# Tariq-Abuhashim/semantic-slam

Hardware: AMD Instinct MI355X
Metric: Mvoxels/sec integrated, 512³ grid @ 640×480 depth; achieved HBM GB/s %peak (higher is better)
Workload: dtype f32

## Files before the change

### include/tsdf_hip_diag.h

```cpp
#ifndef TSDF_HIP_DIAG_H
#define TSDF_HIP_DIAG_H

#include "tsdf_hip.h"

#ifdef __cplusplus
extern "C" {
#endif


int tsdf_integrate_sequence_timed(tsdf_volume *vol, const float *depth_dev, const float *cam2world,
                                  int32_t n_frames, float *elapsed_ms);

int tsdf_integrate_frames_timed(tsdf_volume *vol, const float *const *depth_dev, const uint8_t *const *masks_dev,
                                const float *cam2world, int32_t n_frames, float *elapsed_ms);


int tsdf_probe_graph_replay(tsdf_volume *vol, const float *depth_dev, const float *cam2world, int32_t n_frames,
                            int32_t iters, float *ms_launches, float *ms_graph);

int tsdf_probe_stream(tsdf_volume *vol, int32_t non_temporal, int32_t n_iters, float *elapsed_ms);


int tsdf_selftest_fastdiv(int32_t device, uint64_t seed, uint64_t n_samples, float fx, float cx,
                          uint64_t *mismatches, float first_bad[4]);

int tsdf_selftest_fastdiv_band(int32_t device, uint64_t seed, uint64_t n_samples, uint64_t *mismatches,
                               float first_bad[4]);

int tsdf_selftest_round(int32_t device, uint64_t *mismatches, float first_bad[4]);

int tsdf_selftest_tile_tables(int32_t device, const float *depth_dev, const uint8_t *mask_dev, int32_t im_height,
                              int32_t im_width, float max_depth, uint64_t *mismatches);


int32_t tsdf_frames_per_launch(const tsdf_volume *vol);
int tsdf_shortcut_stats(tsdf_volume *vol, int32_t enable, uint64_t counts_out[3]);
int tsdf_brick_list_stats(tsdf_volume *vol, uint64_t counts_out[4]);
int tsdf_classification_info(tsdf_volume *vol, double info_out[2]);

int tsdf_last_cam2base(const tsdf_volume *vol, float out[16]);


int tsdf_set_kernel_variant(tsdf_volume *vol, int32_t variant);

int tsdf_set_brick_shape(tsdf_volume *vol, int32_t quads, int32_t rows, int32_t slices);
int tsdf_brick_shape(const tsdf_volume *vol, int32_t shape_out[3]);
int tsdf_default_brick_shape(const tsdf_config *cfg, int32_t shape_out[3]);

#ifdef __cplusplus
}
#endif
#endif
```

### semantic_slam_amd/capi.py

```python
import ctypes as C
import os

import numpy as np

_PKG = os.path.dirname(os.path.abspath(__file__))
LIB_PATH = os.environ.get("TSDF_HIP_LIB") or os.path.join(_PKG, "libtsdf_hip.so")

ABI_SYMBOLS = [
    "tsdf_config_default", "tsdf_create", "tsdf_destroy", "tsdf_reset", "tsdf_integrate",
    "tsdf_integrate_u16", "tsdf_convert_depth_u16", "tsdf_set_deferral",
    "tsdf_integrate_device", "tsdf_integrate_cam2base", "tsdf_integrate_masked_device",
    "tsdf_integrate_frames_device",
    "tsdf_sync", "tsdf_download", "tsdf_copy_slices", "tsdf_upload", "tsdf_refresh_summary", "tsdf_device_ptrs", "tsdf_slab_voxels", "tsdf_frames_per_launch", "tsdf_shortcut_stats", "tsdf_brick_list_stats", "tsdf_classification_info",
    "tsdf_get_config", "tsdf_last_cam2base", "tsdf_set_stream", "tsdf_get_stream",
    "tsdf_count_surface", "tsdf_extract_surface", "tsdf_extract_crossings", "tsdf_extract_mesh", "tsdf_save_mesh_ply", "tsdf_save_mesh_welded_ply", "tsdf_save_ply", "tsdf_save_bin", "tsdf_load_bin", "tsdf_save_state", "tsdf_load_state",
    "tsdf_integrate_sequence_timed", "tsdf_integrate_frames_timed", "tsdf_probe_graph_replay", "tsdf_probe_stream", "tsdf_selftest_fastdiv", "tsdf_selftest_fastdiv_band", "tsdf_selftest_round", "tsdf_selftest_tile_tables", "tsdf_set_kernel_variant", "tsdf_set_brick_shape", "tsdf_brick_shape", "tsdf_default_brick_shape", "tsdf_last_error",
    "tsdf_version", "tsdf_multiply_matrix", "tsdf_invert_matrix",
    "tsdf_labels_enable", "tsdf_compose_labels", "tsdf_integrate_labels_device", "tsdf_integrate_frames_labels_device",
    "tsdf_download_labels",
    "tsdf_colour_enable", "tsdf_integrate_colour_device", "tsdf_integrate_rgbd", "tsdf_download_colour",
    "tsdf_raycast_params_default", "tsdf_raycast_device", "tsdf_raycast", "tsdf_batch_raycast_device",
    "tsdf_track_params_default", "tsdf_track", "tsdf_track_system",
    "tsdf_fuse_params_default", "tsdf_fuse_volume",
    "tsdf_associate_params_default", "tsdf_associate_count", "tsdf_associate_assign", "tsdf_batch_associate",
    "tsdf_segment_params_default", "tsdf_segmenter_create", "tsdf_segmenter_destroy", "tsdf_segmenter_set_stream",
    "tsdf_segment_depth_device", "tsdf_segment_refine_masks_device", "tsdf_segment_frame",
    "tsdf_object_origin", "tsdf_batch_create", "tsdf_batch_destroy", "tsdf_batch_size", "tsdf_batch_volume",
    "tsdf_batch_integrate_device", "tsdf_batch_sync",
    "tsdf_group_create", "tsdf_group_destroy", "tsdf_group_size", "tsdf_group_voxels", "tsdf_group_volume",
    "tsdf_group_integrate", "tsdf_group_integrate_frames", "tsdf_group_set_deferral", "tsdf_group_sync", "tsdf_group_reset", "tsdf_group_download",
    "tsdf_group_extract_surface", "tsdf_group_extract_crossings", "tsdf_group_extract_mesh",
    "tsdf_group_save_ply", "tsdf_group_save_mesh_ply", "tsdf_group_save_bin",
]
DIAG_SYMBOLS = [
    "tsdf_integrate_sequence_timed", "tsdf_integrate_frames_timed",
    "tsdf_probe_graph_replay", "tsdf_probe_stream",
    "tsdf_selftest_fastdiv", "tsdf_selftest_fastdiv_band", "tsdf_selftest_round", "tsdf_selftest_tile_tables",
    "tsdf_shortcut_stats", "tsdf_brick_list_stats", "tsdf_classification_info", "tsdf_frames_per_launch", "tsdf_last_cam2base",
    "tsdf_set_kernel_variant", "tsdf_set_brick_shape", "tsdf_brick_shape", "tsdf_default_brick_shape",
]


class TsdfError(RuntimeError):
    pass


SHIPPED_VARIANTS = (0, 1, 3, 7, 8)


def experiments_build():
    return b"+experiments" in load().tsdf_version()


def variants(*wanted):
    exp = experiments_build()
    return [v for v in wanted if v in SHIPPED_VARIANTS or exp]


class TsdfConfig(C.Structure):
    _fields_ = [
        ("im_height", C.c_int32), ("im_width", C.c_int32),
        ("dim_x", C.c_int32), ("dim_y", C.c_int32), ("dim_z", C.c_int32),
        ("z_begin", C.c_int32), ("z_end", C.c_int32),
        ("voxel_size", C.c_float), ("trunc_margin", C.c_float), ("max_depth", C.c_float),
        ("origin", C.c_float * 3), ("cam_K", C.c_float * 9), ("base2world", C.c_float * 16),
        ("device", C.c_int32), ("id", C.c_int32),
    ]


class RaycastParams(C.Structure):
    _fields_ = [
# ... 57 lines not shown
        raise TsdfError(f"{LIB_PATH} not built: run `python -c 'import __graft_entry__ as g; g.build()'` "
                        "(there is no CPU fallback)")
    try:
        import torch
    except ImportError:
        pass
    L = C.CDLL(LIB_PATH)
    vp, f32p, i64p = C.c_void_p, C.POINTER(C.c_float), C.POINTER(C.c_int64)
    L.tsdf_config_default.argtypes = [C.POINTER(TsdfConfig), C.c_int32, C.c_int32]
    L.tsdf_create.argtypes = [C.POINTER(TsdfConfig), C.POINTER(vp)]
    L.tsdf_destroy.argtypes = [vp]
    L.tsdf_reset.argtypes = [vp]
    L.tsdf_integrate.argtypes = [vp, vp, vp]
    L.tsdf_set_deferral.argtypes = [vp, C.c_int32]
    L.tsdf_integrate_u16.argtypes = [vp, vp, C.c_float, C.c_int32, C.c_int32, vp]
    L.tsdf_convert_depth_u16.argtypes = [vp, vp, vp, C.c_float, C.c_int32, C.c_int32]
    L.tsdf_integrate_device.argtypes = [vp, vp, vp]
    L.tsdf_integrate_cam2base.argtypes = [vp, vp, vp]
    L.tsdf_integrate_masked_device.argtypes = [vp, vp, vp, vp]
    L.tsdf_integrate_frames_device.argtypes = [vp, vp, vp, vp, C.c_int32]
    L.tsdf_sync.argtypes = [vp]
    L.tsdf_download.argtypes = [vp, vp, vp]
    L.tsdf_upload.argtypes = [vp, vp, vp]
    L.tsdf_copy_slices.argtypes = [vp, C.c_int32, C.c_int32, vp, vp]
    L.tsdf_refresh_summary.argtypes = [vp]
    L.tsdf_device_ptrs.argtypes = [vp, C.POINTER(vp), C.POINTER(vp)]
    L.tsdf_slab_voxels.argtypes = [vp]
    L.tsdf_slab_voxels.restype = C.c_int64
    L.tsdf_frames_per_launch.argtypes = [vp]
    L.tsdf_frames_per_launch.restype = C.c_int32
    L.tsdf_shortcut_stats.argtypes = [vp, C.c_int32, vp]
    L.tsdf_classification_info.argtypes = [vp, vp]
    L.tsdf_brick_list_stats.argtypes = [vp, vp]
    L.tsdf_get_config.argtypes = [vp, C.POINTER(TsdfConfig)]
    L.tsdf_last_cam2base.argtypes = [vp, vp]
    L.tsdf_set_stream.argtypes = [vp, vp]
    L.tsdf_get_stream.argtypes = [vp, C.POINTER(vp)]
    L.tsdf_count_surface.argtypes = [vp, C.c_float, i64p]
    L.tsdf_extract_surface.argtypes = [vp, C.c_float, vp, C.c_int64, i64p]
    L.tsdf_extract_crossings.argtypes = [vp, vp, vp, C.c_float, vp, C.c_int64, i64p]
    L.tsdf_extract_mesh.argtypes = [vp, vp, vp, C.c_float, vp, C.c_int64, i64p]
    L.tsdf_save_mesh_ply.argtypes = [vp, C.c_char_p, C.c_float]
    L.tsdf_save_mesh_welded_ply.argtypes = [vp, C.c_char_p, C.c_float]
    L.tsdf_save_ply.argtypes = [vp, C.c_char_p, C.c_float]
    L.tsdf_save_bin.argtypes = [vp, C.c_char_p]
    L.tsdf_load_bin.argtypes = [vp, C.c_char_p]
    L.tsdf_save_state.argtypes = [vp, C.c_char_p]
    L.tsdf_load_state.argtypes = [vp, C.c_char_p]
    L.tsdf_integrate_sequence_timed.argtypes = [vp, vp, vp, C.c_int32, f32p]
    L.tsdf_integrate_frames_timed.argtypes = [vp, vp, vp, vp, C.c_int32, f32p]
    L.tsdf_probe_graph_replay.argtypes = [vp, vp, vp, C.c_int32, C.c_int32, f32p, f32p]
    L.tsdf_probe_stream.argtypes = [vp, C.c_int32, C.c_int32, f32p]
    L.tsdf_selftest_fastdiv.argtypes = [C.c_int32, C.c_uint64, C.c_uint64, C.c_float, C.c_float, C.POINTER(C.c_uint64), f32p]
    L.tsdf_selftest_fastdiv_band.argtypes = [C.c_int32, C.c_uint64, C.c_uint64, C.POINTER(C.c_uint64), f32p]
    L.tsdf_selftest_round.argtypes = [C.c_int32, C.POINTER(C.c_uint64), f32p]
    L.tsdf_selftest_tile_tables.argtypes = [C.c_int32, vp, vp, C.c_int32, C.c_int32, C.c_float, C.POINTER(C.c_uint64)]
    L.tsdf_set_kernel_variant.argtypes = [vp, C.c_int32]
    L.tsdf_set_brick_shape.argtypes = [vp, C.c_int32, C.c_int32, C.c_int32]
    L.tsdf_brick_shape.argtypes = [vp, C.POINTER(C.c_int32)]
    L.tsdf_default_brick_shape.argtypes = [C.POINTER(TsdfConfig), C.POINTER(C.c_int32)]
    L.tsdf_last_error.restype = C.c_char_p
    L.tsdf_version.restype = C.c_char_p
    L.tsdf_multiply_matrix.argtypes = [vp, vp, vp]
    L.tsdf_multiply_matrix.restype = None
    L.tsdf_invert_matrix.argtypes = [vp, vp]
    L.tsdf_labels_enable.argtypes = [vp, C.c_float]
# ... 277 lines not shown

    def close(self):
        if self._h:
            if self._owned:
                self.lib.tsdf_destroy(self._h)
            self._h = C.c_void_p()

    def __enter__(self):
        return self

    def __exit__(self, *exc):
        self.close()

    def __del__(self):
        try:
            self.close()
        except Exception:
            pass

    @property
    def n_voxels(self):
        return int(self.lib.tsdf_slab_voxels(self._h))

    def shortcut_stats(self, enable=True):
        out = (C.c_uint64 * 3)()
        check(self.lib.tsdf_shortcut_stats(self._h, 1 if enable else 0, out), "tsdf_shortcut_stats")
        return tuple(int(x) for x in out)

    def brick_list_stats(self):
        out = (C.c_uint64 * 4)()
        check(self.lib.tsdf_brick_list_stats(self._h, out), "tsdf_brick_list_stats")
        return tuple(int(x) for x in out)

    def classification_info(self):
        out = (C.c_double * 2)()
        check(self.lib.tsdf_classification_info(self._h, out), "tsdf_classification_info")
        return float(out[0]), int(out[1])

    @property
    def frames_per_launch(self):
        return int(self.lib.tsdf_frames_per_launch(self._h))

    @property
    def slab_shape(self):
        c = self.cfg
        return (c.z_end - c.z_begin, c.dim_y, c.dim_x)

    def device_ptrs(self):
        t, w = C.c_void_p(), C.c_void_p()
        check(self.lib.tsdf_device_ptrs(self._h, C.byref(t), C.byref(w)), "tsdf_device_ptrs")
        return t.value, w.value

    def integrate(self, depth_host, cam2world):
        d = _f32(depth_host, self.cfg.im_height * self.cfg.im_width)
        p = _f32(cam2world, 16)
        check(self.lib.tsdf_integrate(self._h, d.ctypes.data, p.ctypes.data), "tsdf_integrate")

    def set_deferral(self, n_frames):
        check(self.lib.tsdf_set_deferral(self._h, n_frames), "tsdf_set_deferral")

    def integrate_u16(self, raw_u16, cam2world, depth_factor=5000.0, row_step=1, col_step=1):
        r = np.ascontiguousarray(raw_u16, dtype=np.uint16).ravel()
        if r.size != self.cfg.im_height * self.cfg.im_width:
            raise ValueError("raw frame size does not match the configured image")
        p = _f32(cam2world, 16)
        check(self.lib.tsdf_integrate_u16(self._h, r.ctypes.data, depth_factor, row_step, col_step, p.ctypes.data),
# ... 440 lines not shown
```

### semantic_slam_amd/csrc/tsdf_capi.hip

```cpp
#include "../../include/tsdf_hip.h"
#include "../../include/tsdf_hip_diag.h"

#include <hip/hip_runtime.h>

#include <algorithm>
#include <cmath>
#include <cstdarg>
#include <cstdio>
#include <cstdlib>
#include <cstring>
#include <new>
#include <string>
#include <unordered_map>
#include <vector>

#include "pose_math.h"
#include "host_derive.h"
#include "host_copy.h"
#include "hip_owned.h"
#include "frame_store.h"
#include "tsdf_kernels.hip.h"
#include "tsdf_multiframe.hip.h"
#include "tsdf_labels.hip.h"
#include "tsdf_colour.hip.h"
// ... 83 lines not shown
    HostPtr<tsdfk::FramePose> h_frames[kStageSlots];
    DevPtr<tsdfk::FramePose> d_frames[kStageSlots];
    Event frames_done[kStageSlots];
    bool frames_used[kStageSlots] = {};
    int frames_next = 0;
#endif
    DevPtr<uint16_t> d_label;
    DevPtr<float> d_fp, d_bp;
    float prob_thd = 0.0f;
    DevPtr<uint32_t> d_colour;
    DevPtr<uint8_t> d_rgb[kStageSlots];
    HostPtr<uint8_t> h_rgb[kStageSlots];
    Event rgb_done[kStageSlots];
    bool rgb_used[kStageSlots] = {};
    int rgb_next = 0;
    DevPtr<uint32_t> d_flags;
    size_t n_flags = 0;
    int nseg = 0;
    int chunks_per_slice = 0;
    bool flat = false;
    int brick_q = 0, brick_r = 0, brick_s = 0;
    int tile = 0;
    bool fine_tables = false;
    bool flags_known_zero = false;
#ifdef TSDF_EXPERIMENTS
    DevPtr<unsigned int> d_super;
    size_t super_words = 0;
#endif
    DevPtr<uint4> d_work;
    size_t work_entries = 0;
    int64_t work_nsuper = 0, work_bucket_supers = 0;
    int work_wedge_mode = -1;
    DevPtr<unsigned int> d_shortcut_stats;
    DevPtr<unsigned long long> d_claims;
    HostPtr<unsigned long long> h_claims;
    Event claims_done;
    Stream pre_stream, rb_stream;
    int rb_parity = -1;
    Event pre_done[2], list_free[2], seq_ready;
    int list_parity = 0;
    bool list_used[2] = {false, false};
    bool pipeline_ok = false;
    bool claims_pending = false, claims_known = false;
    double claims_total = 0.0;
    double claim_fraction = 0.0;
    int launches_unclassified = 0;
    DevPtr<char> d_scratch;
    size_t scratch_bytes = 0;
    DevPtr<uint8_t> d_wg_class;
    size_t wg_class_bytes = 0;
    DevPtr<char> d_list;
    size_t list_bytes = 0;
    DevPtr<char> d_track;
    size_t track_bytes = 0;
    HostPtr<tsdfk::TrackState> h_track;
    DevPtr<unsigned long long> d_fuse;
    HostPtr<unsigned long long> h_fuse;
    Event fuse_src_ready, fuse_done;
};

using tsdf_host::kBatchSideStreams;

struct tsdf_batch {
    int device = 0;
    std::vector<tsdf_volume *> vols;
    Stream stream;
// ... 493 lines not shown
        bl.wedge_mode = kWedgeMode;
#ifdef TSDF_EXPERIMENTS
        if (const char *e = std::getenv("TSDF_WEDGE_MODE")) bl.wedge_mode = std::atoi(e);
#endif
        bl.super_h = tsdfk::kSuperBY * mi.common.brick_r;
        bl.super_d = tsdfk::kSuperBZ * mi.common.brick_s;
        bl.wedge_oy = (int)std::lround(std::fmax(-30000.0, std::fmin(30000.0, (double)c.origin[1] / c.voxel_size)));
        bl.wedge_oz = (int)std::lround(std::fmax(-30000.0, std::fmin(30000.0, (double)c.origin[2] / c.voxel_size + c.z_begin)));
        bl.fy_px = (int)std::lround(std::fmax(1.0, std::fmin(16000.0, std::fabs((double)c.cam_K[4]))));
        if (!(c.voxel_size > 0) || std::isnan(c.origin[1]) || std::isnan(c.origin[2])) bl.wedge_mode = 0;
        n_super = (int64_t)bl.nsx * bl.nsy * bl.nsz;
        if (v->work_nsuper != n_super || v->work_wedge_mode != bl.wedge_mode) {
            std::vector<int64_t> per((size_t)tsdfk::kListBuckets, 0);
            for (int64_t id = 0; id < n_super; ++id) {
                const int sz = (int)(id % bl.nsz), sx = (int)((id / bl.nsz) % bl.nsx), sy = (int)((id / bl.nsz) / bl.nsx);
                ++per[(size_t)tsdfk::list_bucket((unsigned int)id, sx, sy, sz, bl)];
            }
            v->work_bucket_supers = *std::max_element(per.begin(), per.end());
            v->work_nsuper = n_super;
            v->work_wedge_mode = bl.wedge_mode;
        }
        cap = v->work_bucket_supers * tsdfk::kSuperBricks;
        const int64_t total = cap * tsdfk::kListBuckets;
        if (total > 0x7fffffffll - 1024) return fail(TSDF_ERR_INVALID, "fused launch: %lld bricks exceed the work list's 32-bit index", (long long)total);
        if (v->work_entries < (size_t)total) {
            if (v->d_work) {
                if (v->pre_stream) HIP_TRY(hipStreamSynchronize(v->pre_stream));
                HIP_TRY(hipStreamSynchronize(v->stream));
            }
            v->work_entries = 0;
            HIP_TRY(dev_alloc(v->d_work, (v->pipeline_ok ? 2 : 1) * (size_t)total * sizeof(uint4)));
            v->work_entries = (size_t)total;
        }
    }
    const hipStream_t ps = pipelined ? v->pre_stream : v->stream;
    auto unwind = [&](int code) {
        if (pipelined && hipEventRecord(v->pre_done[P], ps) == hipSuccess) (void)hipStreamWaitEvent(v->stream, v->pre_done[P], 0);
        (void)tables_end(v);
        return code;
    };
    if (pipelined) {
        HIP_TRY_OR(unwind, hipStreamWaitEvent(ps, inputs_ready, 0));
        if (v->list_used[P]) HIP_TRY_OR(unwind, hipStreamWaitEvent(ps, v->list_free[P], 0));
        if (v->rb_parity == P) HIP_TRY_OR(unwind, hipStreamWaitEvent(ps, v->claims_done, 0));
    } else if (classify && v->rb_parity == P) {
        HIP_TRY(hipStreamWaitEvent(v->stream, v->claims_done, 0));
    }
    if (count_claims) mi.common.claim_counter = claims_p + 1;
    if (classify) {
        const size_t per_frame = tsdf_host::tile_table_elems(mi.common.tiles_w, mi.common.tiles_h);
        float2 *tiles = nullptr;
        int rc = tables_begin(v, &tiles, ps);
        if (rc) return unwind(rc);
        float2 *fine = v->fine_tables ? tiles + (size_t)tsdfk::kMaxFramesPerLaunch * per_frame : nullptr;
        rc = build_tile_tables(ps, c, mi.common, depth_dev, masks_dev, n, tiles, claims_p, fine, pipelined);
        if (rc) return unwind(rc);
        mi.common.fine = fine;
        for (int f = 0; f < n; ++f) mi.frames[f].tiles = tiles + (size_t)f * per_frame;
        for (int f = n; f < tsdfk::kMaxFramesPerLaunch; ++f) mi.frames[f] = mi.frames[0];
    }
    double claims_total = 0.0;
    bool launched = false;
#ifdef TSDF_EXPERIMENTS
    {
        int rc = launch_multi_experiment(v, mi, depth_dev, masks_dev, c2b, n, label_ims != nullptr, any_mask, classify, &launched, &claims_total);
        if (rc) return unwind(rc);
    }
#endif
    if (listed) {
        const int64_t per_group = (int64_t)mi.common.brick_groups * mi.common.bricks_per_group;
        uint4 *const work_p = v->d_work + (size_t)P * v->work_entries;
        bl.list = work_p;
        bl.counters = reinterpret_cast<unsigned char *>(claims_p);
        bl.bucket_cap = (unsigned int)cap;
        bl.poses = reinterpret_cast<tsdfk::ClassPoseTable *>(bl.counters + tsdfk::kCounterBytes);
        hipLaunchKernelGGL(tsdfk::classify_brick_list, dim3((unsigned)((n_super + 3) / 4)), block, 0, ps, mi, bl);
        if (pipelined) {
            HIP_TRY_OR(unwind, hipEventRecord(v->pre_done[P], ps));
            HIP_TRY_OR(unwind, hipStreamWaitEvent(v->stream, v->pre_done[P], 0));
        }
        const dim3 grid_list((unsigned)(((cap + 3) / 4 + 1) * tsdfk::kListBuckets));
        const uint4 *wl = work_p;
        const unsigned char *wc = bl.counters;
        const tsdfk::ClassPoseTable *wp = bl.poses;
        if (label_ims)
            hipLaunchKernelGGL((tsdfk::integrate_brick_list<kBrickNT, true, false>), grid_list, block, 0, v->stream, mi, wl, wc, bl.bucket_cap, wp);
        else if (any_mask)
            hipLaunchKernelGGL((tsdfk::integrate_brick_list<kBrickNT, false, true>), grid_list, block, 0, v->stream, mi, wl, wc, bl.bucket_cap, wp);
        else
            hipLaunchKernelGGL((tsdfk::integrate_brick_list<kBrickNT, false, false>), grid_list, block, 0, v->stream, mi, wl, wc, bl.bucket_cap, wp);
        claims_total = (double)per_group * nz_groups * n;
        launched = true;
    }
    if (!launched) {
        dim3 grid_flat((v->chunks_per_slice + 3) / 4, 1, nz), grid_rows((mi.common.xgroups + 63) / 64, (c.dim_y + 3) / 4, nz);
        const dim3 &g0 = v->flat ? grid_flat : grid_rows;
        if (g0.x > 65535u) mi.z_fastest = 0;
        if (mi.z_fastest) {
            std::swap(grid_flat.x, grid_flat.z);
            std::swap(grid_rows.x, grid_rows.z);
        }
        if (label_ims && v->flat)
            hipLaunchKernelGGL((tsdfk::integrate_multi_inline<1, true, true, true, false>), grid_flat, block, 0, v->stream, mi);
        else if (label_ims)
            hipLaunchKernelGGL((tsdfk::integrate_multi_inline<1, true, false, true, false>), grid_rows, block, 0, v->stream, mi);
        else if (v->flat && any_mask)
            hipLaunchKernelGGL((tsdfk::integrate_multi_inline<1, true, true, false, true>), grid_flat, block, 0, v->stream, mi);
        else if (v->flat)
            hipLaunchKernelGGL((tsdfk::integrate_multi_inline<1, true, true, false, false>), grid_flat, block, 0, v->stream, mi);
// ... 2478 lines not shown
```

### semantic_slam_amd/csrc/tsdf_diag.hip.h

```cpp
#pragma once

namespace {

template <typename Queue>
int time_on_stream(tsdf_volume *v, const char *who, float *elapsed_ms, Queue &&queue)
{
    Event e0, e1;
    HIP_TRY(event_create(e0, hipEventDefault));
    HIP_TRY(event_create(e1, hipEventDefault));
    HIP_TRY(hipEventRecord(e0, v->stream));
    const int rc = queue();
    hipError_t er = hipEventRecord(e1, v->stream);
    hipError_t es = hipEventSynchronize(e1);
    float ms = 0.f;
    hipError_t et = hipEventElapsedTime(&ms, e0, e1);
    if (rc) return rc;
    if (er != hipSuccess || es != hipSuccess || et != hipSuccess)
        return fail(TSDF_ERR_HIP, "%s: event timing failed", who);
    *elapsed_ms = ms;
    return TSDF_OK;
}

int frames_timed(tsdf_volume *v, const float *const *depth_dev, const uint8_t *const *masks_dev,
                 const float *cam2world, int32_t n_frames, float *elapsed_ms, const char *who)
// ... 234 lines not shown
                                   d_c, tw, th, (unsigned long long *)nullptr, d_a, fw, fh);
                e = hipGetLastError();
                if (e == hipSuccess) e = hipDeviceSynchronize();
            }
            if (e == hipSuccess) e = hipGetLastError();
            if (e == hipSuccess) e = hipDeviceSynchronize();
            if (e == hipSuccess) e = hipMemcpy(a.data(), d_a, per * sizeof(float2), hipMemcpyDeviceToHost);
            if (e == hipSuccess) for (size_t i = 0; i < per; ++i) bad += std::memcmp(&a[i], &b[i], sizeof(float2)) != 0;
        }
        if (e != hipSuccess) return fail(TSDF_ERR_HIP, "tsdf_selftest_tile_tables (fine): %s", hipGetErrorString(e));
    }
    *mismatches = bad;
    return TSDF_OK;
}


int32_t tsdf_frames_per_launch(const tsdf_volume *v)
{
    if (!v) return 0;
    return can_fuse(v) ? frames_per_launch(v) : 1;
}

int tsdf_shortcut_stats(tsdf_volume *v, int32_t enable, uint64_t counts_out[3])
{
    if (!v) return fail(TSDF_ERR_INVALID, "tsdf_shortcut_stats: NULL handle");
    int rc = bind_device(v);
    if (rc) return rc;
    HIP_TRY(hipStreamSynchronize(v->stream));
    if (counts_out) {
        unsigned int h[3] = {0, 0, 0};
        if (v->d_shortcut_stats) HIP_TRY(hipMemcpy(h, v->d_shortcut_stats, sizeof h, hipMemcpyDeviceToHost));
        for (int i = 0; i < 3; ++i) counts_out[i] = h[i];
    }
    if (enable && !v->d_shortcut_stats) HIP_TRY(dev_alloc(v->d_shortcut_stats, 8 * sizeof(unsigned int)));
    if (v->d_shortcut_stats) {
        if (enable) HIP_TRY(hipMemset(v->d_shortcut_stats, 0, 8 * sizeof(unsigned int)));
        else v->d_shortcut_stats.reset();
    }
    return TSDF_OK;
}

int tsdf_brick_list_stats(tsdf_volume *v, uint64_t counts_out[4])
{
    if (!v || !counts_out) return fail(TSDF_ERR_INVALID, "tsdf_brick_list_stats: NULL argument");
    int rc = bind_device(v);
    if (rc) return rc;
    HIP_TRY(hipStreamSynchronize(v->stream));
    unsigned int h[8] = {0, 0, 0, 0, 0, 0, 0, 0};
    if (v->d_shortcut_stats) HIP_TRY(hipMemcpy(h, v->d_shortcut_stats, sizeof h, hipMemcpyDeviceToHost));
    for (int i = 0; i < 4; ++i) counts_out[i] = h[3 + i];
    return TSDF_OK;
}

int tsdf_classification_info(tsdf_volume *v, double info_out[2])
{
    if (!v || !info_out) return fail(TSDF_ERR_INVALID, "tsdf_classification_info: NULL argument");
    int rc = bind_device(v);
    if (rc) return rc;
    HIP_TRY(hipStreamSynchronize(v->stream));
    if (v->rb_stream) HIP_TRY(hipStreamSynchronize(v->rb_stream));
    if (v->claims_pending && hipEventQuery(v->claims_done) == hipSuccess) {
        v->claim_fraction = claims_read_back(v);
        v->claims_pending = false;
        v->claims_known = true;
    }
    info_out[0] = v->claims_known ? v->claim_fraction : -1.0;
    info_out[1] = (double)v->launches_unclassified;
    return TSDF_OK;
}

int tsdf_last_cam2base(const tsdf_volume *v, float out[16])
{
    if (!v || !out) return fail(TSDF_ERR_INVALID, "tsdf_last_cam2base: NULL argument");
    std::memcpy(out, v->last_cam2base, sizeof v->last_cam2base);
    return TSDF_OK;
}


int tsdf_set_kernel_variant(tsdf_volume *v, int32_t variant)
{
    if (!v) return fail(TSDF_ERR_INVALID, "tsdf_set_kernel_variant: NULL handle");
    if (!variant_of(variant).known)
        return fail(TSDF_ERR_INVALID, "tsdf_set_kernel_variant: unknown variant %d (this build knows 0, 1, 3, 7, 8%s)", variant,
// ... 36 lines not shown
```

### semantic_slam_amd/csrc/tsdf_multiframe.hip.h

```cpp
#pragma once
#include "tsdf_kernels.hip.h"

namespace tsdfk {

constexpr int kMaxFramesPerLaunch = 32;
constexpr int kFineTile = 4;
constexpr int kFineLevels = 3;
__host__ __device__ inline size_t fine_table_elems(int fw, int fh) { return (size_t)kFineLevels * kFineLevels * fw * fh; }

struct FramePose {
    const float *depth;
    const uint8_t *mask;
    float rx0, ry0, rx1, ry1, rx2, ry2, rz0, rz1, rz2, tz, tx, ty;
    int fast_ok;
    float cz_margin;
    const uint16_t *label_im;
    const float *score_im;
    const float2 *tiles;
    float cz_short;
    float cz_pad;
};

constexpr int kListBuckets = 64;
constexpr int kBucketStride = 256;
// ... 942 lines not shown
}

#ifndef TSDF_BRICK_WAVES
#define TSDF_BRICK_WAVES 8
#endif
template <int R, bool NT, bool FLAT, bool LABELS = false, bool MASKS = true>
__global__ __launch_bounds__(256, R == 2 ? 6 : 1) void integrate_multi_inline(MultiParamsInline mp)
{
    typedef const char __attribute__((address_space(4))) *kernarg_ptr;
    kernarg_ptr base = (kernarg_ptr)__builtin_amdgcn_kernarg_segment_ptr();
    typedef const FramePose __attribute__((address_space(4))) *frames_ptr;
    frames_ptr frames = (frames_ptr)(base + offsetof(MultiParamsInline, frames));
    const int wg_x = mp.z_fastest ? (int)blockIdx.z : (int)blockIdx.x, wg_y = (int)blockIdx.y;
    int wg_z = mp.z_fastest ? (int)blockIdx.x : (int)blockIdx.z;
    if (mp.z_fastest == 2) {
        wg_z += (int)((unsigned)(wg_x + wg_y) % gridDim.x);
        if (wg_z >= (int)gridDim.x) wg_z -= (int)gridDim.x;
    }
    multi_body<R, NT, FLAT, LABELS, MASKS>(mp.common, (const FramePose *)frames, mp.n_frames, wg_x, wg_y, wg_z, mp.labels);
}

constexpr int kSuperBX = 4, kSuperBY = 2, kSuperBZ = 1;
constexpr int kSuperBricks = kSuperBX * kSuperBY * kSuperBZ;
static_assert(kSuperBricks <= 32, "one lane of a half-wave per brick of the super-brick");
constexpr unsigned int kBrickUndecided = 0x80000000u;

struct BrickListParams {
    uint4 *list;
    unsigned char *counters;
    unsigned int bucket_cap;
    ClassPoseTable *poses;
    int nsx, nsy, nsz;
    int wedge_mode, wedge_oy, wedge_oz, super_h, super_d, fy_px;
};

__host__ __device__ inline unsigned int list_bucket(const unsigned int id, const int sx, const int sy, const int sz, const BrickListParams &bl)
{
    const unsigned int h = id * 2654435761u;
    if (bl.wedge_mode == 0) return h >> 26;
    const int yc = bl.wedge_oy + (2 * sy + 1) * bl.super_h / 2;
    int zc = bl.wedge_oz + (2 * sz + 1) * bl.super_d / 2;
    if (zc < 1) zc = 1;
    int t = (yc * 256) / zc;
    t = t > 65536 ? 65536 : (t < -65536 ? -65536 : t);
    const int stripe = (t * bl.fy_px) >> (bl.wedge_mode == 3 ? 11 : 12);
    const int rot = bl.wedge_mode >= 2 ? 3 * (sx >> 2) : 0;
    return ((h >> 29) << 3) | ((unsigned int)(stripe + rot) & 7u);
}

__global__ __launch_bounds__(256) void classify_brick_list(MultiParamsInline mp, BrickListParams bl)
{
    typedef const char __attribute__((address_space(4))) *kernarg_ptr;
    kernarg_ptr base = (kernarg_ptr)__builtin_amdgcn_kernarg_segment_ptr();
    const FramePose *frames = (const FramePose *)(base + offsetof(MultiParamsInline, frames));
    const IntegrateParams &p = mp.common;
    const int id = (int)blockIdx.x * 4 + __builtin_amdgcn_readfirstlane((int)threadIdx.y), lane = threadIdx.x;
    if (id >= bl.nsx * bl.nsy * bl.nsz) return;
    const int sz = id % bl.nsz, t = id / bl.nsz, sx = t % bl.nsx, sy = t / bl.nsx;
    const int nzg = (p.nz + p.brick_s - 1) / p.brick_s;
    const int i0 = sx * kSuperBX, g0 = sy * kSuperBY, zg0 = sz * kSuperBZ;
    const int i1 = min(i0 + kSuperBX, p.bricks_per_group) - 1, g1 = min(g0 + kSuperBY, p.brick_groups) - 1, zg1 = min(zg0 + kSuperBZ, nzg) - 1;
    const unsigned int frames_mask = mp.n_frames >= 32 ? 0xffffffffu : ((1u << mp.n_frames) - 1u);
    static_assert(kMaxFramesPerLaunch == 32, "one frame per lane of a half-wave");
    const int xa = i0 * p.brick_q * 4, xb = (i1 + 1) * p.brick_q * 4 - 1;
    const int ya = g0 * p.brick_r, yb = min((g1 + 1) * p.brick_r, p.dim_y) - 1;
    const int z0 = zg0 * p.brick_s, z1 = min((zg1 + 1) * p.brick_s, p.nz) - 1;
    const ClassPose mine_q = class_pose(frames[lane & 31]);
    if (id == 0 && lane < kMaxFramesPerLaunch) class_pose_store(bl.poses, lane, mine_q);
    const float2 *fine_f = p.fine != nullptr ? p.fine + (size_t)(lane & 31) * fine_table_elems(p.fine_w, p.fine_h) : nullptr;
    const int cls = classify_patch<true>(p, mine_q, xa, xb, ya, yb, p.z_begin + z0, p.z_begin + z1, fine_f);
    const unsigned int super_free = (unsigned int)__ballot(cls == 1) & frames_mask;
    const unsigned int super_skip = (unsigned int)__ballot(cls == 2) & frames_mask;
    const int n_in = (i1 - i0 + 1) * (g1 - g0 + 1) * (zg1 - zg0 + 1);
    static_assert(kListBuckets == 64, "six bits: list_bucket");
    const unsigned int bkt = list_bucket((unsigned int)id, sx, sy, sz, bl);
    unsigned char *bucket = bl.counters + (size_t)bkt * kBucketStride;
    if (lane == 0) {
        if (p.claim_counter != nullptr && (super_free | super_skip) != 0u)
            atomicAdd(reinterpret_cast<unsigned long long *>(bucket + 8),
                      ((unsigned long long)(n_in * __popc(super_free)) << 32) | (unsigned long long)(n_in * __popc(super_skip)));
        if (p.shortcut_stats != nullptr) {
            if (super_skip == frames_mask) { atomicAdd(p.shortcut_stats + 2, (unsigned)(n_in * mp.n_frames)); atomicAdd(p.shortcut_stats + 3, 1u); }
            else {
                atomicAdd(p.shortcut_stats + 4, (unsigned)n_in);
                if ((super_free | super_skip) != frames_mask) atomicAdd(p.shortcut_stats + 5, (unsigned)n_in);
            }
        }
    }
    if (super_skip == frames_mask) return;
    const int k = lane;
    const int i = i0 + k % kSuperBX, g = g0 + (k / kSuperBX) % kSuperBY, zg = zg0 + k / (kSuperBX * kSuperBY);
    const bool mine = k < kSuperBricks && i <= i1 && g <= g1 && zg <= zg1;
    const unsigned long long live_mask = __ballot(mine);
    const unsigned int undecided = (super_free | super_skip) != frames_mask ? kBrickUndecided : 0u;
    const unsigned int n_live = (unsigned)__popcll(live_mask);
    unsigned int at = 0u;
    if (lane == 0) at = atomicAdd(reinterpret_cast<unsigned int *>(bucket) + (undecided ? 0 : 1), n_live);
    at = __builtin_amdgcn_readfirstlane(at);
    at = bkt * bl.bucket_cap + (undecided ? at : bl.bucket_cap - at - n_live);
    if (mine)
        bl.list[at + (unsigned)__popcll(live_mask & ((1ull << lane) - 1ull))] =
            make_uint4((unsigned)(g * p.bricks_per_group + i) | undecided, (unsigned)zg, super_free, super_skip);
}

template <bool NT, bool LABELS, bool MASKS>
__global__ __launch_bounds__(256, LABELS ? 6 : TSDF_BRICK_WAVES) void integrate_brick_list(MultiParamsInline mp, const uint4 *__restrict__ list,
                                                                                          const unsigned char *__restrict__ counters,
                                                                                          const unsigned int bucket_cap,
                                                                                          const ClassPoseTable *__restrict__ poses)
{
    typedef const char __attribute__((address_space(4))) *kernarg_ptr;
    kernarg_ptr base = (kernarg_ptr)__builtin_amdgcn_kernarg_segment_ptr();
    const FramePose *frames = (const FramePose *)(base + offsetof(MultiParamsInline, frames));
    const unsigned int b = blockIdx.x % kListBuckets, grp = blockIdx.x / kListBuckets;
    const unsigned int wave = (unsigned)__builtin_amdgcn_readfirstlane((int)threadIdx.y);
    const uint2 n = *reinterpret_cast<const uint2 *>(counters + (size_t)b * kBucketStride);
    const unsigned int front_groups = (n.x + 3u) / 4u;
    unsigned int at;
    if (grp < front_groups) {
        at = grp * 4u + wave;
        if (at >= n.x) return;
    } else {
        const unsigned int k = (grp - front_groups) * 4u + wave;
        if (k >= n.y) return;
        at = bucket_cap - 1u - k;
    }
    const uint4 e = list[(size_t)b * bucket_cap + at];
    const int brick = (int)(e.x & ~kBrickUndecided), zg = (int)e.y;
    unsigned int free_frames = e.z, skip_frames = e.w;
    if (e.x & kBrickUndecided) {
        const IntegrateParams &p = mp.common;
        const int lane = threadIdx.x;
        const unsigned int frames_mask = mp.n_frames >= 32 ? 0xffffffffu : ((1u << mp.n_frames) - 1u);
        const int g = brick / p.bricks_per_group, i = brick - g * p.bricks_per_group;
        const int xa = i * p.brick_q * 4, ya = g * p.brick_r;
// ... 77 lines not shown
```

Baseline: 405,400.

## Refine undecided super-bricks per brick in classify prepass before listing

When a super-brick has few undecided frames (up to four rounds of four frames), the classify kernel now reclassifies each of its eight bricks against those frames in the prepass. It records exact per-brick free/skip masks, drops bricks that every frame skips, and lists the rest as decided instead of undecided. This aims to cut per-voxel work and fallback handling in the integrate kernel, at the cost of extra classification rounds in the prepass. Also adds a selftest kernel and stats histograms to validate the refinement.

```diff
diff --git a/include/tsdf_hip_diag.h b/include/tsdf_hip_diag.h
--- a/include/tsdf_hip_diag.h
+++ b/include/tsdf_hip_diag.h
@@ -32,10 +32,13 @@
 int tsdf_selftest_tile_tables(int32_t device, const float *depth_dev, const uint8_t *mask_dev, int32_t im_height,
                               int32_t im_width, float max_depth, uint64_t *mismatches);
 
+int tsdf_selftest_prepass(tsdf_volume *vol, int32_t enable, uint64_t counts_out[2]);
+
 
 int32_t tsdf_frames_per_launch(const tsdf_volume *vol);
 int tsdf_shortcut_stats(tsdf_volume *vol, int32_t enable, uint64_t counts_out[3]);
 int tsdf_brick_list_stats(tsdf_volume *vol, uint64_t counts_out[4]);
+int tsdf_prepass_pair_stats(tsdf_volume *vol, uint64_t counts_out[44]);
 int tsdf_classification_info(tsdf_volume *vol, double info_out[2]);
 
 int tsdf_last_cam2base(const tsdf_volume *vol, float out[16]);
diff --git a/semantic_slam_amd/capi.py b/semantic_slam_amd/capi.py
--- a/semantic_slam_amd/capi.py
+++ b/semantic_slam_amd/capi.py
@@ -11,7 +11,7 @@
     "tsdf_integrate_u16", "tsdf_convert_depth_u16", "tsdf_set_deferral",
     "tsdf_integrate_device", "tsdf_integrate_cam2base", "tsdf_integrate_masked_device",
     "tsdf_integrate_frames_device",
-    "tsdf_sync", "tsdf_download", "tsdf_copy_slices", "tsdf_upload", "tsdf_refresh_summary", "tsdf_device_ptrs", "tsdf_slab_voxels", "tsdf_frames_per_launch", "tsdf_shortcut_stats", "tsdf_brick_list_stats", "tsdf_classification_info",
+    "tsdf_sync", "tsdf_download", "tsdf_copy_slices", "tsdf_upload", "tsdf_refresh_summary", "tsdf_device_ptrs", "tsdf_slab_voxels", "tsdf_frames_per_launch", "tsdf_shortcut_stats", "tsdf_brick_list_stats", "tsdf_prepass_pair_stats", "tsdf_selftest_prepass", "tsdf_classification_info",
     "tsdf_get_config", "tsdf_last_cam2base", "tsdf_set_stream", "tsdf_get_stream",
     "tsdf_count_surface", "tsdf_extract_surface", "tsdf_extract_crossings", "tsdf_extract_mesh", "tsdf_save_mesh_ply", "tsdf_save_mesh_welded_ply", "tsdf_save_ply", "tsdf_save_bin", "tsdf_load_bin", "tsdf_save_state", "tsdf_load_state",
     "tsdf_integrate_sequence_timed", "tsdf_integrate_frames_timed", "tsdf_probe_graph_replay", "tsdf_probe_stream", "tsdf_selftest_fastdiv", "tsdf_selftest_fastdiv_band", "tsdf_selftest_round", "tsdf_selftest_tile_tables", "tsdf_set_kernel_variant", "tsdf_set_brick_shape", "tsdf_brick_shape", "tsdf_default_brick_shape", "tsdf_last_error",
@@ -36,7 +36,7 @@
     "tsdf_integrate_sequence_timed", "tsdf_integrate_frames_timed",
     "tsdf_probe_graph_replay", "tsdf_probe_stream",
     "tsdf_selftest_fastdiv", "tsdf_selftest_fastdiv_band", "tsdf_selftest_round", "tsdf_selftest_tile_tables",
-    "tsdf_shortcut_stats", "tsdf_brick_list_stats", "tsdf_classification_info", "tsdf_frames_per_launch", "tsdf_last_cam2base",
+    "tsdf_shortcut_stats", "tsdf_brick_list_stats", "tsdf_prepass_pair_stats", "tsdf_selftest_prepass", "tsdf_classification_info", "tsdf_frames_per_launch", "tsdf_last_cam2base",
     "tsdf_set_kernel_variant", "tsdf_set_brick_shape", "tsdf_brick_shape", "tsdf_default_brick_shape",
 ]
 
@@ -160,6 +160,8 @@
     L.tsdf_shortcut_stats.argtypes = [vp, C.c_int32, vp]
     L.tsdf_classification_info.argtypes = [vp, vp]
     L.tsdf_brick_list_stats.argtypes = [vp, vp]
+    L.tsdf_prepass_pair_stats.argtypes = [vp, vp]
+    L.tsdf_selftest_prepass.argtypes = [vp, C.c_int32, vp]
     L.tsdf_get_config.argtypes = [vp, C.POINTER(TsdfConfig)]
     L.tsdf_last_cam2base.argtypes = [vp, vp]
     L.tsdf_set_stream.argtypes = [vp, vp]
@@ -503,6 +505,17 @@
         check(self.lib.tsdf_brick_list_stats(self._h, out), "tsdf_brick_list_stats")
         return tuple(int(x) for x in out)
 
+    def prepass_pair_stats(self):
+        out = (C.c_uint64 * 44)()
+        check(self.lib.tsdf_prepass_pair_stats(self._h, out), "tsdf_prepass_pair_stats")
+        v = [int(x) for x in out]
+        return v[0], v[1], v[2], {u: v[2 + u] for u in range(1, 33)}, {n: v[35 + n] for n in range(9)}
+
+    def selftest_prepass(self, enable=True):
+        out = (C.c_uint64 * 2)()
+        check(self.lib.tsdf_selftest_prepass(self._h, 1 if enable else 0, out), "tsdf_selftest_prepass")
+        return int(out[0]), int(out[1])
+
     def classification_info(self):
         out = (C.c_double * 2)()
         check(self.lib.tsdf_classification_info(self._h, out), "tsdf_classification_info")
diff --git a/semantic_slam_amd/csrc/tsdf_capi.hip b/semantic_slam_amd/csrc/tsdf_capi.hip
--- a/semantic_slam_amd/csrc/tsdf_capi.hip
+++ b/semantic_slam_amd/csrc/tsdf_capi.hip
@@ -139,6 +139,9 @@
     int64_t work_nsuper = 0, work_bucket_supers = 0;
     int work_wedge_mode = -1;
     DevPtr<unsigned int> d_shortcut_stats;
+    DevPtr<unsigned long long> d_prepass_bad;
+    DevPtr<uint4> d_prepass_check;
+    size_t prepass_check_bricks = 0;
     DevPtr<unsigned long long> d_claims;
     HostPtr<unsigned long long> h_claims;
     Event claims_done;
@@ -698,6 +701,18 @@
             HIP_TRY(dev_alloc(v->d_work, (v->pipeline_ok ? 2 : 1) * (size_t)total * sizeof(uint4)));
             v->work_entries = (size_t)total;
         }
+        bl.check = nullptr;
+        if (v->d_prepass_bad) {
+            const size_t bricks = (size_t)mi.common.brick_groups * mi.common.bricks_per_group * (size_t)nz_groups;
+            if (v->prepass_check_bricks < bricks) {
+                if (v->pre_stream) HIP_TRY(hipStreamSynchronize(v->pre_stream));
+                HIP_TRY(hipStreamSynchronize(v->stream));
+                v->prepass_check_bricks = 0;
+                HIP_TRY(dev_alloc(v->d_prepass_check, bricks * sizeof(uint4)));
+                v->prepass_check_bricks = bricks;
+            }
+            bl.check = v->d_prepass_check;
+        }
     }
     const hipStream_t ps = pipelined ? v->pre_stream : v->stream;
     auto unwind = [&](int code) {
@@ -740,7 +755,11 @@
         bl.counters = reinterpret_cast<unsigned char *>(claims_p);
         bl.bucket_cap = (unsigned int)cap;
         bl.poses = reinterpret_cast<tsdfk::ClassPoseTable *>(bl.counters + tsdfk::kCounterBytes);
+        if (bl.check) HIP_TRY_OR(unwind, hipMemsetAsync(bl.check, 0, (size_t)per_group * nz_groups * sizeof(uint4), ps));
         hipLaunchKernelGGL(tsdfk::classify_brick_list, dim3((unsigned)((n_super + 3) / 4)), block, 0, ps, mi, bl);
+        if (bl.check)
+            hipLaunchKernelGGL(tsdfk::selftest_prepass_check, dim3((unsigned)((per_group * nz_groups + 3) / 4)), block, 0, ps, mi, bl,
+                               (unsigned long long *)v->d_prepass_bad);
         if (pipelined) {
             HIP_TRY_OR(unwind, hipEventRecord(v->pre_done[P], ps));
             HIP_TRY_OR(unwind, hipStreamWaitEvent(v->stream, v->pre_done[P], 0));
diff --git a/semantic_slam_amd/csrc/tsdf_diag.hip.h b/semantic_slam_amd/csrc/tsdf_diag.hip.h
--- a/semantic_slam_amd/csrc/tsdf_diag.hip.h
+++ b/semantic_slam_amd/csrc/tsdf_diag.hip.h
@@ -290,9 +290,9 @@
         if (v->d_shortcut_stats) HIP_TRY(hipMemcpy(h, v->d_shortcut_stats, sizeof h, hipMemcpyDeviceToHost));
         for (int i = 0; i < 3; ++i) counts_out[i] = h[i];
     }
-    if (enable && !v->d_shortcut_stats) HIP_TRY(dev_alloc(v->d_shortcut_stats, 8 * sizeof(unsigned int)));
+    if (enable && !v->d_shortcut_stats) HIP_TRY(dev_alloc(v->d_shortcut_stats, tsdfk::kStatWords * sizeof(unsigned int)));
     if (v->d_shortcut_stats) {
-        if (enable) HIP_TRY(hipMemset(v->d_shortcut_stats, 0, 8 * sizeof(unsigned int)));
+        if (enable) HIP_TRY(hipMemset(v->d_shortcut_stats, 0, tsdfk::kStatWords * sizeof(unsigned int)));
         else v->d_shortcut_stats.reset();
     }
     return TSDF_OK;
@@ -307,6 +307,48 @@
     unsigned int h[8] = {0, 0, 0, 0, 0, 0, 0, 0};
     if (v->d_shortcut_stats) HIP_TRY(hipMemcpy(h, v->d_shortcut_stats, sizeof h, hipMemcpyDeviceToHost));
     for (int i = 0; i < 4; ++i) counts_out[i] = h[3 + i];
+    return TSDF_OK;
+}
+
+int tsdf_prepass_pair_stats(tsdf_volume *v, uint64_t counts_out[44])
+{
+    if (!v || !counts_out) return fail(TSDF_ERR_INVALID, "tsdf_prepass_pair_stats: NULL argument");
+    int rc = bind_device(v);
+    if (rc) return rc;
+    HIP_TRY(hipStreamSynchronize(v->stream));
+    unsigned int h[tsdfk::kStatWords] = {};
+    if (v->d_shortcut_stats) HIP_TRY(hipMemcpy(h, v->d_shortcut_stats, sizeof h, hipMemcpyDeviceToHost));
+    static_assert(tsdfk::kSuperBricks == 8, "counts_out: 3 + 32 + 9 numbers");
+    counts_out[0] = tsdfk::kPrepassMaxRounds;
+    counts_out[1] = tsdfk::kRoundFrames;
+    counts_out[2] = h[tsdfk::kStatFallback];
+    for (int u = 1; u <= 32; ++u) counts_out[2 + u] = h[tsdfk::kStatHistU + u];
+    for (int n = 0; n <= tsdfk::kSuperBricks; ++n) counts_out[35 + n] = h[tsdfk::kStatHistLive + n];
+    return TSDF_OK;
+}
+
+int tsdf_selftest_prepass(tsdf_volume *v, int32_t enable, uint64_t counts_out[2])
+{
+    if (!v) return fail(TSDF_ERR_INVALID, "tsdf_selftest_prepass: NULL handle");
+    int rc = bind_device(v);
+    if (rc) return rc;
+    rc = flush_pending(v);
+    if (rc) return rc;
+    if (v->pre_stream) HIP_TRY(hipStreamSynchronize(v->pre_stream));
+    HIP_TRY(hipStreamSynchronize(v->stream));
+    if (counts_out) {
+        unsigned long long h[2] = {0, 0};
+        if (v->d_prepass_bad) HIP_TRY(hipMemcpy(h, v->d_prepass_bad, sizeof h, hipMemcpyDeviceToHost));
+        counts_out[0] = h[0]; counts_out[1] = h[1];
+    }
+    if (enable) {
+        if (!v->d_prepass_bad) HIP_TRY(dev_alloc(v->d_prepass_bad, 2 * sizeof(unsigned long long)));
+        HIP_TRY(hipMemset(v->d_prepass_bad, 0, 2 * sizeof(unsigned long long)));
+    } else {
+        v->d_prepass_bad.reset();
+        v->d_prepass_check.reset();
+        v->prepass_check_bricks = 0;
+    }
     return TSDF_OK;
 }
 
diff --git a/semantic_slam_amd/csrc/tsdf_multiframe.hip.h b/semantic_slam_amd/csrc/tsdf_multiframe.hip.h
--- a/semantic_slam_amd/csrc/tsdf_multiframe.hip.h
+++ b/semantic_slam_amd/csrc/tsdf_multiframe.hip.h
@@ -998,6 +998,7 @@
     ClassPoseTable *poses;
     int nsx, nsy, nsz;
     int wedge_mode, wedge_oy, wedge_oz, super_h, super_d, fy_px;
+    uint4 *check;
 };
 
 __host__ __device__ inline unsigned int list_bucket(const unsigned int id, const int sx, const int sy, const int sz, const BrickListParams &bl)
@@ -1014,59 +1015,185 @@
     return ((h >> 29) << 3) | ((unsigned int)(stripe + rot) & 7u);
 }
 
-__global__ __launch_bounds__(256) void classify_brick_list(MultiParamsInline mp, BrickListParams bl)
+constexpr size_t kBrickListParamsOffset = (sizeof(MultiParamsInline) + alignof(BrickListParams) - 1) / alignof(BrickListParams) * alignof(BrickListParams);
+constexpr int kRoundFrames = 32 / kSuperBricks;
+constexpr int kPrepassMaxRounds = 4;
+static_assert(kRoundFrames >= 1 && kRoundFrames * kSuperBricks == 32, "a round fills the half-wave");
+constexpr int kStatFallback = 7, kStatHistU = 8, kStatHistLive = kStatHistU + 33, kStatWords = 64;
+static_assert(kStatHistLive + kSuperBricks + 1 <= kStatWords, "the histograms fit the block");
+
+constexpr unsigned int kCheckNone = 0u, kCheckFallback = 1u, kCheckListed = 2u, kCheckDropped = 3u;
+
+__global__ __launch_bounds__(256, 8) void classify_brick_list(MultiParamsInline mp, BrickListParams bl)
+{
+    typedef const char __attribute__((address_space(4))) *kernarg_ptr;
+    kernarg_ptr base = (kernarg_ptr)__builtin_amdgcn_kernarg_segment_ptr();
+    const FramePose *frames = (const FramePose *)(base + offsetof(MultiParamsInline, frames));
+    auto params = [&]() -> const IntegrateParams & {
+        kernarg_ptr b = base;
+        asm volatile("" : "+s"(b));
+        return *(const IntegrateParams *)(b + offsetof(MultiParamsInline, common));
+    };
+    const IntegrateParams &p0 = params();
+    const int id = (int)blockIdx.x * 4 + __builtin_amdgcn_readfirstlane((int)threadIdx.y), lane = threadIdx.x;
+    if (id >= bl.nsx * bl.nsy * bl.nsz) return;
+    const int sz = id % bl.nsz, t = id / bl.nsz, sx = t % bl.nsx, sy = t / bl.nsx;
+    const int nzg = (p0.nz + p0.brick_s - 1) / p0.brick_s;
+    const int i0 = sx * kSuperBX, g0 = sy * kSuperBY, zg0 = sz * kSuperBZ;
+    const int i1 = min(i0 + kSuperBX, p0.bricks_per_group) - 1, g1 = min(g0 + kSuperBY, p0.brick_groups) - 1, zg1 = min(zg0 + kSuperBZ, nzg) - 1;
+    const unsigned int frames_mask = mp.n_frames >= 32 ? 0xffffffffu : ((1u << mp.n_frames) - 1u);
+    static_assert(kMaxFramesPerLaunch == 32, "one frame per lane of a half-wave");
+    const int n_in = (i1 - i0 + 1) * (g1 - g0 + 1) * (zg1 - zg0 + 1);
+    static_assert(kListBuckets == 64, "six bits: list_bucket");
+    const unsigned int bkt = list_bucket((unsigned int)id, sx, sy, sz, bl);
+    unsigned char *bucket = bl.counters + (size_t)bkt * kBucketStride;
+    const int k = (lane & 31) % kSuperBricks, jj = (lane & 31) / kSuperBricks;
+    const int i = i0 + k % kSuperBX, g = g0 + (k / kSuperBX) % kSuperBY, zg = zg0 + k / (kSuperBX * kSuperBY);
+    const bool live = i <= i1 && g <= g1 && zg <= zg1;
+    const bool mine = lane < kSuperBricks && live;
+    int xa = i0 * p0.brick_q * 4, xb = (i1 + 1) * p0.brick_q * 4 - 1;
+    int ya = g0 * p0.brick_r, yb = min((g1 + 1) * p0.brick_r, p0.dim_y) - 1;
+    int z0 = zg0 * p0.brick_s, z1 = min((zg1 + 1) * p0.brick_s, p0.nz) - 1;
+    int f = lane & 31;
+    unsigned int super_free = 0u, super_skip = 0u, U = 0u, rem = 0u;
+    unsigned int free_k = 0u, skip_k = 0u;
+    unsigned int round_f = 0u;
+    static_assert(kRoundFrames <= 4, "round_f: a byte per frame of the round");
+    bool exact = false;
+#pragma unroll 1
+    for (int round = -1;; ++round) {
+        const IntegrateParams &p = params();
+        const ClassPose q = class_pose(frames[f]);
+        if (round < 0 && id == 0 && lane < kMaxFramesPerLaunch) class_pose_store(bl.poses, lane, q);
+        const float2 *fine_f = p.fine != nullptr ? p.fine + (size_t)f * fine_table_elems(p.fine_w, p.fine_h) : nullptr;
+        const int cls = classify_patch<true>(p, q, xa, xb, ya, yb, p.z_begin + z0, p.z_begin + z1, fine_f);
+        const unsigned int fw = (unsigned int)__ballot(cls == 1), sw = (unsigned int)__ballot(cls == 2);
+        if (round < 0) {
+            super_free = fw & frames_mask;
+            super_skip = sw & frames_mask;
+            U = frames_mask & ~(super_free | super_skip);
+            if (lane == 0) {
+                if (p.claim_counter != nullptr && (super_free | super_skip) != 0u)
+                    atomicAdd(reinterpret_cast<unsigned long long *>(bucket + 8),
+                              ((unsigned long long)(n_in * __popc(super_free)) << 32) | (unsigned long long)(n_in * __popc(super_skip)));
+                if (p.shortcut_stats != nullptr) {
+                    if (super_skip == frames_mask) { atomicAdd(p.shortcut_stats + 2, (unsigned)(n_in * mp.n_frames)); atomicAdd(p.shortcut_stats + 3, 1u); }
+                    else if (U != 0u) {
+                        atomicAdd(p.shortcut_stats + 5, (unsigned)n_in);
+                        atomicAdd(p.shortcut_stats + kStatHistU + __popc(U), 1u);
+                        atomicAdd(p.shortcut_stats + kStatHistLive + n_in, 1u);
+                        if (__popc(U) > kPrepassMaxRounds * kRoundFrames) atomicAdd(p.shortcut_stats + kStatFallback, 1u);
+                    }
+                }
+            }
+            if (super_skip == frames_mask) return;
+            if (U == 0u || __popc(U) > kPrepassMaxRounds * kRoundFrames) break;
+            exact = true;
+            rem = U;
+            const int bi = live ? i : i0, bg = live ? g : g0, bz = live ? zg : zg0;
+            xa = bi * p.brick_q * 4; xb = xa + p.brick_q * 4 - 1;
+            ya = bg * p.brick_r; yb = min(ya + p.brick_r - 1, p.dim_y - 1);
+            z0 = bz * p.brick_s; z1 = min(z0 + p.brick_s - 1, p.nz - 1);
+        } else {
+#pragma unroll
+            for (int j = 0; j < kRoundFrames; ++j) {
+                const unsigned int fj = (round_f >> (8 * j)) & 0xffu;
+                if (fj < 32u) {
+                    const int bit = j * kSuperBricks + k;
+                    free_k |= ((fw >> bit) & 1u) << fj;
+                    skip_k |= ((sw >> bit) & 1u) << fj;
+                }
+            }
+            if (rem == 0u) break;
+        }
+        f = 0;
+        round_f = 0u;
+#pragma unroll
+        for (int j = 0; j < kRoundFrames; ++j) {
+            const unsigned int fj = rem != 0u ? (unsigned)(__ffs((int)rem) - 1) : 32u;
+            rem &= rem - 1u;
+            round_f |= fj << (8 * j);
+            if (jj == j && fj < 32u) f = (int)fj;
+        }
+    }
+    const IntegrateParams &pe = params();
+    kernarg_ptr bl_base = base;
+    asm volatile("" : "+s"(bl_base));
+    const BrickListParams &ble = *(const BrickListParams *)(bl_base + kBrickListParamsOffset);
+    const unsigned int w_free = super_free | free_k, w_skip = super_skip | skip_k;
+    const bool dropped = mine && exact && w_skip == frames_mask;
+    const bool front = mine && !dropped && (exact ? (w_free | w_skip) != frames_mask : U != 0u);
+    const bool back = mine && !dropped && !front;
+    const unsigned long long front_mask = __ballot(front), back_mask = __ballot(back);
+    const unsigned int n_front = (unsigned)__popcll(front_mask), n_back = (unsigned)__popcll(back_mask);
+    const unsigned int undecided = exact ? 0u : (U != 0u ? kBrickUndecided : 0u);
+    unsigned int at_front = 0u, at_back = 0u;
+    if (lane == 0) {
+        if (n_front) at_front = atomicAdd(reinterpret_cast<unsigned int *>(bucket), n_front);
+        if (n_back) at_back = atomicAdd(reinterpret_cast<unsigned int *>(bucket) + 1, n_back);
+        if (pe.shortcut_stats != nullptr) {
+            const unsigned int n_drop = (unsigned)n_in - n_front - n_back;
+            atomicAdd(pe.shortcut_stats + 4, n_front + n_back);
+            if (n_drop) { atomicAdd(pe.shortcut_stats + 2, n_drop * (unsigned)mp.n_frames); atomicAdd(pe.shortcut_stats + 6, n_drop); }
+        }
+    }
+    at_front = __builtin_amdgcn_readfirstlane(at_front);
+    at_back = __builtin_amdgcn_readfirstlane(at_back);
+    const unsigned long long below = (1ull << lane) - 1ull;
+    const unsigned int brick = (unsigned)(g * pe.bricks_per_group + i);
+    if (front)
+        ble.list[bkt * ble.bucket_cap + at_front + (unsigned)__popcll(front_mask & below)] = make_uint4(brick | undecided, (unsigned)zg, w_free, w_skip);
+    if (back)
+        ble.list[bkt * ble.bucket_cap + (ble.bucket_cap - at_back - n_back) + (unsigned)__popcll(back_mask & below)] = make_uint4(brick, (unsigned)zg, w_free, w_skip);
+    if (ble.check != nullptr && mine)
+        ble.check[(size_t)zg * ((size_t)pe.brick_groups * pe.bricks_per_group) + brick] =
+            make_uint4(dropped ? kCheckDropped : (undecided ? kCheckFallback : kCheckListed), w_free, w_skip, U);
+}
+
+__global__ __launch_bounds__(256) void selftest_prepass_check(MultiParamsInline mp, BrickListParams bl, unsigned long long *out)
 {
     typedef const char __attribute__((address_space(4))) *kernarg_ptr;
     kernarg_ptr base = (kernarg_ptr)__builtin_amdgcn_kernarg_segment_ptr();
     const FramePose *frames = (const FramePose *)(base + offsetof(MultiParamsInline, frames));
     const IntegrateParams &p = mp.common;
-    const int id = (int)blockIdx.x * 4 + __builtin_amdgcn_readfirstlane((int)threadIdx.y), lane = threadIdx.x;
-    if (id >= bl.nsx * bl.nsy * bl.nsz) return;
-    const int sz = id % bl.nsz, t = id / bl.nsz, sx = t % bl.nsx, sy = t / bl.nsx;
-    const int nzg = (p.nz + p.brick_s - 1) / p.brick_s;
-    const int i0 = sx * kSuperBX, g0 = sy * kSuperBY, zg0 = sz * kSuperBZ;
-    const int i1 = min(i0 + kSuperBX, p.bricks_per_group) - 1, g1 = min(g0 + kSuperBY, p.brick_groups) - 1, zg1 = min(zg0 + kSuperBZ, nzg) - 1;
+    const int nzg = (p.nz + p.brick_s - 1) / p.brick_s, per_group = p.brick_groups * p.bricks_per_group;
+    const long long idx = (long long)blockIdx.x * 4 + __builtin_amdgcn_readfirstlane((int)threadIdx.y);
+    if (idx >= (long long)nzg * per_group) return;
+    const int lane = threadIdx.x;
+    const int zg = (int)(idx / per_group), brick = (int)(idx - (long long)zg * per_group);
+    const int g = brick / p.bricks_per_group, i = brick - g * p.bricks_per_group;
     const unsigned int frames_mask = mp.n_frames >= 32 ? 0xffffffffu : ((1u << mp.n_frames) - 1u);
-    static_assert(kMaxFramesPerLaunch == 32, "one frame per lane of a half-wave");
-    const int xa = i0 * p.brick_q * 4, xb = (i1 + 1) * p.brick_q * 4 - 1;
-    const int ya = g0 * p.brick_r, yb = min((g1 + 1) * p.brick_r, p.dim_y) - 1;
-    const int z0 = zg0 * p.brick_s, z1 = min((zg1 + 1) * p.brick_s, p.nz) - 1;
-    const ClassPose mine_q = class_pose(frames[lane & 31]);
-    if (id == 0 && lane < kMaxFramesPerLaunch) class_pose_store(bl.poses, lane, mine_q);
+    const ClassPose q = class_pose(frames[lane & 31]);
     const float2 *fine_f = p.fine != nullptr ? p.fine + (size_t)(lane & 31) * fine_table_elems(p.fine_w, p.fine_h) : nullptr;
-    const int cls = classify_patch<true>(p, mine_q, xa, xb, ya, yb, p.z_begin + z0, p.z_begin + z1, fine_f);
-    const unsigned int super_free = (unsigned int)__ballot(cls == 1) & frames_mask;
-    const unsigned int super_skip = (unsigned int)__ballot(cls == 2) & frames_mask;
-    const int n_in = (i1 - i0 + 1) * (g1 - g0 + 1) * (zg1 - zg0 + 1);
-    static_assert(kListBuckets == 64, "six bits: list_bucket");
-    const unsigned int bkt = list_bucket((unsigned int)id, sx, sy, sz, bl);
-    unsigned char *bucket = bl.counters + (size_t)bkt * kBucketStride;
-    if (lane == 0) {
-        if (p.claim_counter != nullptr && (super_free | super_skip) != 0u)
-            atomicAdd(reinterpret_cast<unsigned long long *>(bucket + 8),
-                      ((unsigned long long)(n_in * __popc(super_free)) << 32) | (unsigned long long)(n_in * __popc(super_skip)));
-        if (p.shortcut_stats != nullptr) {
-            if (super_skip == frames_mask) { atomicAdd(p.shortcut_stats + 2, (unsigned)(n_in * mp.n_frames)); atomicAdd(p.shortcut_stats + 3, 1u); }
-            else {
-                atomicAdd(p.shortcut_stats + 4, (unsigned)n_in);
-                if ((super_free | super_skip) != frames_mask) atomicAdd(p.shortcut_stats + 5, (unsigned)n_in);
-            }
-        }
-    }
-    if (super_skip == frames_mask) return;
-    const int k = lane;
-    const int i = i0 + k % kSuperBX, g = g0 + (k / kSuperBX) % kSuperBY, zg = zg0 + k / (kSuperBX * kSuperBY);
-    const bool mine = k < kSuperBricks && i <= i1 && g <= g1 && zg <= zg1;
-    const unsigned long long live_mask = __ballot(mine);
-    const unsigned int undecided = (super_free | super_skip) != frames_mask ? kBrickUndecided : 0u;
-    const unsigned int n_live = (unsigned)__popcll(live_mask);
-    unsigned int at = 0u;
-    if (lane == 0) at = atomicAdd(reinterpret_cast<unsigned int *>(bucket) + (undecided ? 0 : 1), n_live);
-    at = __builtin_amdgcn_readfirstlane(at);
-    at = bkt * bl.bucket_cap + (undecided ? at : bl.bucket_cap - at - n_live);
-    if (mine)
-        bl.list[at + (unsigned)__popcll(live_mask & ((1ull << lane) - 1ull))] =
-            make_uint4((unsigned)(g * p.bricks_per_group + i) | undecided, (unsigned)zg, super_free, super_skip);
+    unsigned int sfree, sskip, bfree, bskip;
+    {
+        const int i0 = i / kSuperBX * kSuperBX, g0 = g / kSuperBY * kSuperBY, zg0 = zg / kSuperBZ * kSuperBZ;
+        const int i1 = min(i0 + kSuperBX, p.bricks_per_group) - 1, g1 = min(g0 + kSuperBY, p.brick_groups) - 1, zg1 = min(zg0 + kSuperBZ, nzg) - 1;
+        const int cls = classify_patch<true>(p, q, i0 * p.brick_q * 4, (i1 + 1) * p.brick_q * 4 - 1, g0 * p.brick_r, min((g1 + 1) * p.brick_r, p.dim_y) - 1,
+                                             p.z_begin + zg0 * p.brick_s, p.z_begin + min((zg1 + 1) * p.brick_s, p.nz) - 1, fine_f);
+        sfree = (unsigned int)__ballot(cls == 1) & frames_mask;
+        sskip = (unsigned int)__ballot(cls == 2) & frames_mask;
+    }
+    {
+        const int xa = i * p.brick_q * 4, ya = g * p.brick_r;
+        const int z0 = zg * p.brick_s, z1 = min(z0 + p.brick_s - 1, p.nz - 1);
+        const int cls = classify_patch<true>(p, q, xa, xa + p.brick_q * 4 - 1, ya, min(ya + p.brick_r - 1, p.dim_y - 1), p.z_begin + z0, p.z_begin + z1, fine_f);
+        bfree = (unsigned int)__ballot(cls == 1) & frames_mask;
+        bskip = (unsigned int)__ballot(cls == 2) & frames_mask;
+    }
+    if (lane != 0) return;
+    const unsigned int U = frames_mask & ~(sfree | sskip);
+    const uint4 rec = bl.check[idx];
+    bool ok;
+    if (sskip == frames_mask) ok = rec.x == kCheckNone;
+    else if (U == 0u) ok = rec.x == kCheckListed && rec.y == sfree && rec.z == sskip && rec.w == 0u;
+    else if (__popc(U) > kPrepassMaxRounds * kRoundFrames) ok = rec.x == kCheckFallback && rec.y == sfree && rec.z == sskip && rec.w == U;
+    else {
+        const unsigned int want_free = sfree | (bfree & U), want_skip = sskip | (bskip & U);
+        ok = rec.x == (want_skip == frames_mask ? kCheckDropped : kCheckListed) && rec.y == want_free && rec.z == want_skip && rec.w == U;
+        atomicAdd(out + 1, 1ull);
+    }
+    if (!ok) atomicAdd(out, 1ull);
 }
 
 template <bool NT, bool LABELS, bool MASKS>
```

After: 405,400 (median of 3 runs). Within noise of the previous version (-0.0%).
